# andrpac/alphazero-gnn

Hardware: AMD Instinct MI355X
Metric: board-state evals/sec (GNN fwd) + self-play games/sec, Connect4, 1/2/4/8 GPU (higher is better)
Workload: dtype f32 (fp16x2 row-scaled split, 3 products: output_transform GEMMs and the trunk's conv2 split each fp32 operand row, power-of-two scaled, into 2 fp16 terms, 3 fp16 MFMA products, fp32 accumulate; ~22-bit operands: tests/test_gpu_trained.py holds pi / v / log pi to 1e-5 of float64 and of the reference; 1 GPU; Connect4 (reference 7x7+pass board) Connect4GNN predict_with_gnn per-board fwd: trunk -> output_transform -> heads, batch of random boards per GPU; global_batch=512, batch_per_gpu=512, feature_dim=3136, parallelism=dp1 (independent shards, no collective)

## Files before the change

### alphazero-gnn_amd/csrc/az_gemm.hip

```cpp
#include <stdio.h>
#include <stdlib.h>
#include <string.h>

#include <algorithm>
#include <atomic>
#include <mutex>
#include <type_traits>
#include <utility>
#include <unordered_map>
#include <vector>

#include "az_common.h"
#include "az_x3.h"
#include "az_heads.h"
#include "az_trunk_split.h"

namespace az {

struct GemmArgs {
  int M, N, K;
  const float* A; int lda;
  const float* A2; int lda2; int K0;
  const int* a_rows;
  const float* B; int ldb;
// ... 3450 lines not shown
      } else {
        f = mt % q.am + q.am * ((col >> 7) % q.an);
        b = q.bf;
        W = q.am * q.an * q.KT;
      }
      const int np = csk_block_of((f + 1) * q.KT - 1, b, W) - csk_block_of(f * q.KT, b, W) + 1;
      for (int pc = 0; pc < np; ++pc)
#pragma unroll
        for (int a = 0; a < HS; ++a) s[a] += st[(cb * he.mp + pc) * HS + a];
    }
  } else {
    if (row >= M) return;
    for (int t = lane; t < P; t += 64)
#pragma unroll
      for (int a = 0; a < HS; ++a) s[a] += src[(size_t)t * HS + a];
  }
#pragma unroll
  for (int a = 0; a < HS; ++a) {
    float v = s[a];
    v += dpp_mov<0xB1>(v);
    v += dpp_mov<0x4E>(v);
    v += dpp_mov<0x141>(v);
    v += dpp_mov<0x140>(v);
    s[a] = (__builtin_bit_cast(float, __builtin_amdgcn_readlane(__builtin_bit_cast(int, v), 0)) +
            __builtin_bit_cast(float, __builtin_amdgcn_readlane(__builtin_bit_cast(int, v), 16)) +
            __builtin_bit_cast(float, __builtin_amdgcn_readlane(__builtin_bit_cast(int, v), 32)) +
            __builtin_bit_cast(float, __builtin_amdgcn_readlane(__builtin_bit_cast(int, v), 48)));
  }
  if (lane != 0) return;
  const int A = he.A;
  float l[8];
  float mx = -INFINITY;
#pragma unroll
  for (int a = 0; a < 8; ++a)
    if (a < A) {
      l[a] = s[a] + he.bp[a];
      mx = fmaxf(mx, l[a]);
    }
  float se = 0.f;
#pragma unroll
  for (int a = 0; a < 8; ++a)
    if (a < A) se += expf(l[a] - mx);
  const float lse = logf(se);
#pragma unroll
  for (int a = 0; a < 8; ++a)
    if (a < A) {
      const float o = (l[a] - mx) - lse;
      he.logp[(size_t)row * A + a] = o;
      if (he.pi) he.pi[(size_t)row * A + a] = expf(o);
    }
  he.v[row] = tanhf(s[8] + he.bv[0]);
}

__global__ __launch_bounds__(256) void c4_w2_frag_kernel(const float* __restrict__ w2,
                                                         float* __restrict__ frag) {
  const int i = blockIdx.x * 256 + threadIdx.x;
  if (i >= 18432) return;
  const int e = i & 3, lane = (i >> 2) & 63, q = (i >> 8) % 18, nt = i / (18 * 256);
  const int st = 4 * q + e, tap = st >> 3, j = st & 7;
  const int co = 16 * nt + (lane & 15), ci = 8 * (lane >> 4) + j;
  frag[i] = w2[co * 288 + ci * 9 + tap];
}

const float* conv2_frags(const float* w2, hipStream_t s) {
  if (!weights_registered(w2, 64, 288, 288)) return nullptr;
  const long gen = g_wgen.load();
  std::lock_guard<std::mutex> lk(g_wmu);
  WScaleEntry* e = wcache_entry(w2, 64, 288, 288);
  if (!e) return nullptr;
  if (!e->frags[0]) {
    if (hipMalloc(&e->frags[0], (size_t)2 * 18432 * sizeof(float)) != hipSuccess) {
      e->frags[0] = nullptr;
      return nullptr;
    }
    e->frags[1] = e->frags[0] + 18432;
    e->fgen = 0;
  }
  if (e->fgen == gen) return e->frags[e->fcur];
  const int nxt = e->fcur ^ 1;
  hipLaunchKernelGGL(c4_w2_frag_kernel, dim3(72), dim3(256), 0, s, w2, e->frags[nxt]);
  if (hipStreamSynchronize(s) != hipSuccess) return nullptr;
  e->fcur = nxt;
  e->fgen = gen;
  return e->frags[nxt];
}

constexpr int COMPOSE_JB = 4;
__global__ __launch_bounds__(1024) void compose_heads_kernel(
    const float* __restrict__ w2, const float* __restrict__ b2, const float* __restrict__ wp,
    const float* __restrict__ bp, const float* __restrict__ wv, const float* __restrict__ bv,
    int F, int A, double* __restrict__ part, float* __restrict__ out) {
  __shared__ double sh[3][16][64];
  const int lane = threadIdx.x & 63;
  const int g = __builtin_amdgcn_readfirstlane((int)(threadIdx.x >> 6));
  if ((int)blockIdx.x == (F + 63) / 64) {
    if (blockIdx.y != 0) return;
    double* ps = &sh[0][0][0];
    double* ps2 = ps + 9 * 256;
    const int t = threadIdx.x;
    if (t < 256) {
      double acc[9];
#pragma unroll
      for (int a = 0; a < 9; ++a) acc[a] = 0.0;
      for (int j = t; j < F; j += 256) {
        const double b = (double)b2[j];
#pragma unroll
        for (int a = 0; a < 8; ++a)
          if (a < A) acc[a] += (double)wp[(size_t)a * F + j] * b;
        acc[8] += (double)wv[j] * b;
      }
#pragma unroll
      for (int a = 0; a < 9; ++a) ps[a * 256 + t] = acc[a];
    }
    __syncthreads();
    if (t < 9 * 16) {
      const int a = t >> 4, q = t & 15;
      double s = 0.0;
      for (int i = 0; i < 16; ++i) s += ps[a * 256 + q * 16 + i];
      ps2[a * 16 + q] = s;
    }
    __syncthreads();
    if (t < 9 && (t < A || t == 8)) {
      double s = 0.0;
      for (int q = 0; q < 16; ++q) s += ps2[t * 16 + q];
      const int row = t == 8 ? A : t;
      out[(size_t)(A + 1) * F + row] = (float)(s + (double)(t == 8 ? bv[0] : bp[t]));
    }
    return;
  }
  const int k = blockIdx.x * 64 + lane;
  const bool kin = k < F;
  const int kc = kin ? k : F - 1;
  double acc[9];
// ... 767 lines not shown
```

### alphazero-gnn_amd/csrc/az_trunk.hip

```cpp
#include <stdlib.h>

#include <algorithm>
#include "az_common.h"
#include "az_heads.h"
#include "az_trunk_split.h"
#include "az_x3.h"

namespace az {

#ifdef AZ_TRUNK_SELFCHECK
__device__ unsigned* g_trunk_chk;
#endif

template <int NB, bool REGW>
constexpr int trunk_union_floats() {
  constexpr int after = NB <= 4 ? NB * 3136 : NB * C1_FLOATS_PER_BOARD;
  return REGW || after >= W2S_FLOATS ? after : W2S_FLOATS;
}

template <int NB, bool REGW>
constexpr int trunk_waves_per_eu() { return REGW && NB <= 3 ? 4 : 1; }
template <int NB, bool REGW>
constexpr int trunk_blocks_per_cu() { return REGW && NB <= 3 ? 2 : 1; }

struct TrunkHeads {
  const float* wp; const float* bp; int A; const float* wv; const float* bv;
  float* logp; float* pi; float* v;
};

template <int NB>
__device__ __forceinline__ void trunk_rows_heads(const float* ob, int nb, int b0,
                                                 const TrunkHeads& hd) {
  constexpr int AMAX = 8, PW = AMAX + 1, K = 3136, NCH = (K + HEADS_KC - 1) / HEADS_KC;
  __shared__ float part[NB][NCH][PW];
  __shared__ float hsm[NB][PW];
  const int tid = threadIdx.x, lane = tid & 63, wave = tid >> 6;
  const int A = hd.A;
  const f32x4 z = {0.f, 0.f, 0.f, 0.f};
  static_assert(NCH <= 16, "two chunks per wave");
  auto load_w = [&](int c, f32x4 (&w)[AMAX + 1], bool& kin, int& kc) {
    const int k = c * HEADS_KC + lane * 4;
    kin = k < K;
    kc = kin ? k : 0;
#pragma unroll
    for (int a = 0; a < AMAX; ++a)
      w[a] = *reinterpret_cast<const f32x4*>(hd.wp + (size_t)min(a, A - 1) * K + kc);
    w[AMAX] = *reinterpret_cast<const f32x4*>(hd.wv + kc);
  };
  auto chunk = [&](int c, f32x4 (&w)[AMAX + 1], bool kin, int kc) {
#pragma unroll
    for (int a = 0; a < AMAX; ++a) w[a] = (a < A && kin) ? w[a] : z;
    w[AMAX] = kin ? w[AMAX] : z;
    float ps[NB], vs[NB];
#pragma unroll
    for (int b = 0; b < NB; ++b) {
      const f32x4 x = kin && b < nb ? *reinterpret_cast<const f32x4*>(ob + b * K + kc) : z;
      float pv[AMAX];
#pragma unroll
      for (int a = 0; a < AMAX; ++a)
        pv[a] = fmaf(x[3], w[a][3], fmaf(x[2], w[a][2], fmaf(x[1], w[a][1], x[0] * w[a][0])));
      ps[b] = wave_multi_sum<AMAX>(pv);
      vs[b] = wave_sum_x(
          fmaf(x[3], w[AMAX][3], fmaf(x[2], w[AMAX][2], fmaf(x[1], w[AMAX][1], x[0] * w[AMAX][0]))));
    }
    const int a = lane >> 3;
#pragma unroll
    for (int b = 0; b < NB; ++b) {
      if (b < nb && (lane & 7) == 0 && a < A) part[b][c][a] = ps[b];
      if (b < nb && lane == 0) part[b][c][A] = vs[b];
    }
  };
  f32x4 w0[AMAX + 1], w1[AMAX + 1];
  bool kin0, kin1 = false;
  int kc0, kc1 = 0;
  const bool two = wave + 8 < NCH;
  load_w(wave, w0, kin0, kc0);
  if (two) load_w(wave + 8, w1, kin1, kc1);
  chunk(wave, w0, kin0, kc0);
  if (two) chunk(wave + 8, w1, kin1, kc1);
  __syncthreads();
  if (tid < NB * PW) {
    const int b = tid / PW, a = tid % PW;
    if (b < nb && a <= A) {
      float s = 0.f;
      for (int c = 0; c < NCH; ++c) s += part[b][c][a];
      hsm[b][a] = s;
    }
  }
  __syncthreads();
  if (tid < nb) {
    const int row = b0 + tid;
    float l[AMAX];
    float mx = -INFINITY;
#pragma unroll
    for (int a = 0; a < AMAX; ++a)
      if (a < A) {
        l[a] = hsm[tid][a] + hd.bp[a];
        mx = fmaxf(mx, l[a]);
      }
    float se = 0.f;
#pragma unroll
    for (int a = 0; a < AMAX; ++a)
      if (a < A) se += expf(l[a] - mx);
    const float lse = logf(se);
#pragma unroll
    for (int a = 0; a < AMAX; ++a)
      if (a < A) {
        const float o = (l[a] - mx) - lse;
        hd.logp[(size_t)row * A + a] = o;
        if (hd.pi) hd.pi[(size_t)row * A + a] = expf(o);
      }
    hd.v[row] = tanhf(hsm[tid][A] + hd.bv[0]);
  }
}

template <int NB, bool HEADS = false, bool REGW = false>
__device__ __forceinline__ void c4_trunk_tile(const int8_t* __restrict__ boards, int B,
                                              const float* __restrict__ w1,
                                              const float* __restrict__ b1,
                                              const float* __restrict__ w2,
                                              const float* __restrict__ b2,
                                              float* __restrict__ feat, float* un,
                                              unsigned short* __restrict__ apl = nullptr,
                                              float* __restrict__ asc = nullptr,
                                              const float* __restrict__ w2f = nullptr,
                                              const TrunkHeads* hd = nullptr) {
  static_assert(!HEADS || NB <= 4, "HEADS: the rows staged in LDS");
  float* const ob = un;
  constexpr int P = 49, PP = 81, CI = 32;
  constexpr int NT = TTILES[NB];
  constexpr bool STAGE = NB <= 4;
  __shared__ float bd[NB * PP + 1];
  __shared__ __attribute__((aligned(16))) float c1s[STAGE ? NB * C1_FLOATS_PER_BOARD : 4];
  float* const c1 = STAGE ? c1s : un;
  __shared__ float w1s[CI * 9 + CI + 1];
  __shared__ float c1wmax[NB][8];
  __shared__ float c1inv[NB];
  const int tid = threadIdx.x;
  const int b0 = blockIdx.x * NB;
  const int nb = min(NB, B - b0);
  const int lane = tid & 63, wave = tid >> 6;
  const int nt = wave & 3, mh = wave >> 2;
  const int h = lane >> 4, c16 = lane & 15;
  const int co = nt * 16 + c16;
  const uint16_t* const rows = trunk_rows<NB>();
  constexpr int NW2 = 64 * 72 / 512;
  f32x4v wst[NW2];
  float breg[72];
  if constexpr (REGW) {
#pragma unroll
    for (int q = 0; q < 18; ++q) {
      const f32x4v v = reinterpret_cast<const f32x4v*>(w2f)[(nt * 18 + q) * 64 + lane];
#pragma unroll
      for (int e = 0; e < 4; ++e) breg[4 * q + e] = v[e];
    }
  } else {
#pragma unroll
    for (int j = 0; j < NW2; ++j) wst[j] = reinterpret_cast<const f32x4v*>(w2)[tid + 512 * j];
  }
  constexpr int NBD = (NB * PP + 511) / 512;
  int8_t bdv[NBD];
  bool bdin[NBD];
#pragma unroll
  for (int j = 0; j < NBD; ++j) {
    const int i = tid + 512 * j;
    const int b = i / PP, pp = i % PP, px = pp / 9, py = pp % 9;
    bdin[j] = i < NB * PP && b < nb && px >= 1 && px <= 7 && py >= 1 && py <= 7;
    bdv[j] = boards[bdin[j] ? (size_t)(b0 + b) * P + (px - 1) * 7 + (py - 1) : (size_t)b0 * P];
  }
  const float w1v = tid < CI * 9 ? w1[tid] : b1[min(tid - CI * 9, CI - 1)];
  const float bias = b2[co];
  __builtin_amdgcn_sched_barrier(0);
  if constexpr (!REGW) {
#pragma unroll
    for (int j = 0; j < NW2; ++j) {
      const int i = tid + 512 * j;
      float* d = un + (i / 72) * W2S_STRIDE + (i % 72) * 4;
      d[0] = wst[j][0]; d[1] = wst[j][1]; d[2] = wst[j][2]; d[3] = wst[j][3];
    }
  }
#pragma unroll
  for (int j = 0; j < NBD; ++j)
    bd[min(tid + 512 * j, NB * PP)] = bdin[j] ? (float)bdv[j] : 0.f;
  w1s[min(tid, CI * 9 + CI)] = w1v;
  __syncthreads();
  if constexpr (!REGW) {
#pragma unroll
    for (int s = 0; s < 72; ++s) {
      const int tap = s >> 3, ci = 8 * h + (s & 7);
      breg[s] = un[co * W2S_STRIDE + ci * 9 + (tap / 3) * 3 + (tap % 3)];
    }
  }
  bf16x8 bh[9], bl[9];
  const float iw = w2_planes(breg, bh, bl);
  if constexpr (!STAGE && !REGW) __syncthreads();
  constexpr int NI = NB * PP * 4, NIT = (NI + 511) / 512;
  float cv[NIT][8];
  float cm[NB];
#pragma unroll
  for (int b = 0; b < NB; ++b) cm[b] = 0.f;
#pragma unroll
  for (int it = 0; it < NIT; ++it) {
    const int i = tid + 512 * it;
    if (i < NI) {
      const int b = i / (PP * 4), r = i - b * (PP * 4);
      conv1_octet(w1s, bd + b * PP, r >> 2, r & 3, cv[it]);
      const float m = octet_max(cv[it]);
#pragma unroll
      for (int q = 0; q < NB; ++q)
        if (q == b) cm[q] = fmaxf(cm[q], m);
    }
  }
#pragma unroll
  for (int b = 0; b < NB; ++b) {
#pragma unroll
    for (int o = 32; o > 0; o >>= 1) cm[b] = fmaxf(cm[b], __shfl_xor(cm[b], o));
    if (lane == 0) c1wmax[b][wave] = cm[b];
  }
  __syncthreads();
#pragma unroll
  for (int it = 0; it < NIT; ++it) {
    const int i = tid + 512 * it;
    if (i < NI) {
      const int b = i / (PP * 4), r = i - b * (PP * 4);
      float mx = c1wmax[b][0];
#pragma unroll
      for (int w = 1; w < 8; ++w) mx = fmaxf(mx, c1wmax[b][w]);
      float inv;
      const float sa = h3_scale(mx, H3_TA, &inv);
      c1_store(c1 + b * C1_FLOATS_PER_BOARD, r >> 2, r & 3, cv[it], sa);
      if (r == 0) c1inv[b] = inv;
    }
  }
  __syncthreads();
#ifdef AZ_TRUNK_SELFCHECK
  auto c1_check = [&](int phase, int i) {
    if (i >= NI || !g_trunk_chk) return;
    const int b = i / (PP * 4), r = i - b * (PP * 4);
    float v[8], v2[8];
    conv1_octet(w1s, bd + b * PP, r >> 2, r & 3, v);
    asm volatile("" ::: "memory");
    conv1_octet(w1s, bd + b * PP, r >> 2, r & 3, v2);
    float mx = c1wmax[b][0];
    for (int w = 1; w < 8; ++w) mx = fmaxf(mx, c1wmax[b][w]);
    float inv;
    const float sa = h3_scale(mx, H3_TA, &inv);
    u32x4 o[2];
    split2s(f32x4{v[0], v[1], v[2], v[3]}, f32x4{v[4], v[5], v[6], v[7]}, sa, o);
    const u32x4* u = reinterpret_cast<const u32x4*>(c1 + b * C1_FLOATS_PER_BOARD) +
                     C1_UNITS_PER_POS * (r >> 2) + (r & 3);
    const u32x4 x0 = u[0], x1 = u[4];
    int nbad = 0, nconv = 0;
    for (int e = 0; e < 4; ++e) nbad += (x0[e] != o[0][e]) + (x1[e] != o[1][e]);
    for (int e = 0; e < 8; ++e) nconv += __float_as_uint(v[e]) != __float_as_uint(v2[e]);
    if (nbad || nconv) {
      const unsigned k = atomicAdd(g_trunk_chk, 1u);
      if (k < 2048) {
        unsigned* d = g_trunk_chk + 64 + 48 * k;
        d[0] = blockIdx.x; d[1] = tid; d[2] = i; d[3] = phase;
        d[4] = nbad; d[5] = nconv;
        d[6] = __builtin_amdgcn_s_getreg((4) | (0 << 6) | ((32 - 1) << 11));
        d[7] = __float_as_uint(sa);
        for (int e = 0; e < 4; ++e) {
          d[8 + e] = x0[e]; d[12 + e] = x1[e];
          d[16 + e] = o[0][e]; d[20 + e] = o[1][e];
        }
        for (int e = 0; e < 8; ++e) {
          d[24 + e] = __float_as_uint(v[e]);
          d[32 + e] = __float_as_uint(v2[e]);
        }
      }
    }
  };
#pragma unroll
  for (int it = 0; it < NIT; ++it) c1_check(0, tid + 512 * it);
  c1_check(1, (tid + 192) % (NIT * 512));
#endif

  const u32x4* const c1u = reinterpret_cast<const u32x4*>(c1);
  auto a_unit = [&](int mt) { return mt < NT ? c1_row_unit(rows[16 * mt + c16] & 0x7fff, h) : h; };
  float bm[NB];
#pragma unroll
  for (int b = 0; b < NB; ++b) bm[b] = 0.f;
  auto store_tile = [&](int mt, const f32x4v& acc) {
#pragma unroll
    for (int r = 0; r < 4; ++r) {
      const int e = rows[16 * mt + h * 4 + r];
      const int b = (e & 0x7fff) / P, p = (e & 0x7fff) - P * ((e & 0x7fff) / P);
      if (!(e & 0x8000) && b < nb) {
        const float v = acc[r] * (c1inv[b] * iw) + bias;
        const float o = v > 0.f ? v : 0.f;
        if constexpr (STAGE) {
          ob[b * 3136 + co * P + p] = o;
#pragma unroll
          for (int q = 0; q < NB; ++q)
            if (q == b) bm[q] = fmaxf(bm[q], o);
        } else {
          feat[(size_t)(b0 + b) * 3136 + co * P + p] = o;
        }
      }
    }
  };
  for (int mt = mh; mt < NT; mt += 4) {
    const int u0 = a_unit(mt), u1 = a_unit(mt + 2);
    f32x4v acc0 = {0.f, 0.f, 0.f, 0.f}, acc1 = {0.f, 0.f, 0.f, 0.f};
#pragma unroll
    for (int tap = 0; tap < 9; ++tap) {
      const int off = c1_tap_units(tap);
      const u32x4 ah0 = c1u[u0 + off], al0 = c1u[u0 + off + 4];
      const u32x4 ah1 = c1u[u1 + off], al1 = c1u[u1 + off + 4];
      acc0 = conv2_step(ah0, al0, bh[tap], bl[tap], acc0);
      acc1 = conv2_step(ah1, al1, bh[tap], bl[tap], acc1);
    }
    store_tile(mt, acc0);
    if (mt + 2 < NT) store_tile(mt + 2, acc1);
  }
  if constexpr (STAGE) {
    __shared__ float wmax[NB][8];
    if (apl) {
#pragma unroll
      for (int b = 0; b < NB; ++b) {
#pragma unroll
        for (int o = 32; o > 0; o >>= 1) bm[b] = fmaxf(bm[b], __shfl_xor(bm[b], o));
        if (lane == 0) wmax[b][wave] = bm[b];
      }
    }
    __syncthreads();
#ifdef AZ_TRUNK_SELFCHECK
#pragma unroll
    for (int it = 0; it < NIT; ++it) c1_check(2, tid + 512 * it);
#endif
    f32x4v* dst = feat ? reinterpret_cast<f32x4v*>(feat + (size_t)b0 * 3136) : nullptr;
    const f32x4v* src = reinterpret_cast<const f32x4v*>(ob);
    if (!apl) {
      for (int i = tid; i < nb * 784; i += 512) dst[i] = src[i];
      return;
    }
    for (int ch = tid; ch < nb * 392; ch += 512) {
      const int b = ch / 392, c = ch - b * 392;
      float mx = wmax[b][0];
#pragma unroll
      for (int w = 1; w < 8; ++w) mx = fmaxf(mx, wmax[b][w]);
      float inv;
      const float sc = h3_scale(mx, H3_TA, &inv);
      const f32x4v lo = src[2 * ch], hi = src[2 * ch + 1];
      if (dst) {
        dst[2 * ch] = lo;
        dst[2 * ch + 1] = hi;
      }
      u32x4 o[2];
      split2s(__builtin_bit_cast(f32x4, lo), __builtin_bit_cast(f32x4, hi), sc, o);
      *reinterpret_cast<u32x4*>(apl + p2_chunk(b0 + b, c, 0, 3136)) = o[0];
      *reinterpret_cast<u32x4*>(apl + p2_chunk(b0 + b, c, 1, 3136)) = o[1];
      if (c == 0) {
        asc[b0 + b] = sc;
        asc[B + b0 + b] = inv;
      }
    }
    if constexpr (HEADS) trunk_rows_heads<NB>(ob, nb, b0, *hd);
  }
}

#define AZ_TRUNK_LB(NB_, REGW_)                                                                  \
  __attribute__((amdgpu_flat_work_group_size(1, 512),                                            \
                 amdgpu_waves_per_eu(trunk_waves_per_eu<NB_, REGW_>())))
template <int NB, bool REGW = false>
__global__ AZ_TRUNK_LB(NB, REGW) void c4_trunk_kernel(const int8_t* __restrict__ boards, int B,
                                                      const float* __restrict__ w1,
                                                      const float* __restrict__ b1,
                                                      const float* __restrict__ w2,
                                                      const float* __restrict__ b2,
                                                      float* __restrict__ feat,
                                                      const float* __restrict__ w2f = nullptr) {
  __shared__ __attribute__((aligned(16))) float un[trunk_union_floats<NB, REGW>()];
  c4_trunk_tile<NB, false, REGW>(boards, B, w1, b1, w2, b2, feat, un, nullptr, nullptr, w2f);
}

template <int NB, bool HEADS = false, bool REGW = false>
__global__ AZ_TRUNK_LB(NB, REGW) void c4_trunk_split_a_kernel(
    const int8_t* __restrict__ boards, int B, const float* __restrict__ w1,
    const float* __restrict__ b1, const float* __restrict__ w2, const float* __restrict__ b2,
    float* __restrict__ feat, unsigned short* __restrict__ apl, float* __restrict__ asc,
    const float* __restrict__ w2f = nullptr, TrunkHeads hd = {}) {
  static_assert(NB <= 4, "the A split reads the LDS staging tile");
  __shared__ __attribute__((aligned(16))) float un[trunk_union_floats<NB, REGW>()];
  c4_trunk_tile<NB, HEADS, REGW>(boards, B, w1, b1, w2, b2, feat, un, apl, asc, w2f, &hd);
}

template <bool IN_I8>
__global__ __launch_bounds__(256) void conv3x3_relu_kernel(const void* __restrict__ in_, int B,
                                                          int Cin, int H, int W,
                                                          const float* __restrict__ w,
                                                          const float* __restrict__ b, int Cout,
                                                          int pad, float* __restrict__ out) {
  const int Ho = H + 2 * pad - 2, Wo = W + 2 * pad - 2;
  const long total = (long)B * Cout * Ho * Wo;
  for (long idx = blockIdx.x * 256L + threadIdx.x; idx < total; idx += (long)gridDim.x * 256) {
    const int xo = idx % Wo, yo = (idx / Wo) % Ho, co = (idx / ((long)Wo * Ho)) % Cout;
    const long bi = idx / ((long)Wo * Ho * Cout);
    float s = 0.f;
    for (int ci = 0; ci < Cin; ++ci) {
#pragma unroll
      for (int kh = 0; kh < 3; ++kh) {
        const int yi = yo + kh - pad;
        if (yi < 0 || yi >= H) continue;
#pragma unroll
        for (int kw = 0; kw < 3; ++kw) {
          const int xi = xo + kw - pad;
          if (xi < 0 || xi >= W) continue;
          const long ii = ((bi * Cin + ci) * H + yi) * W + xi;
          const float iv = IN_I8 ? (float)static_cast<const int8_t*>(in_)[ii]
                                 : static_cast<const float*>(in_)[ii];
          s = fmaf(w[((co * Cin + ci) * 3 + kh) * 3 + kw], iv, s);
        }
      }
    }
    s += b[co];
    out[idx] = s > 0.f ? s : 0.f;
  }
}

constexpr int HEADS_ROWS = 16;

template <int AMAX>
__global__ __launch_bounds__(256) void heads_partial_kernel(
    const float* __restrict__ hp, int ldhp, const float* __restrict__ hv, int ldhv, int B, int K,
    const float* __restrict__ wp, int A, const float* __restrict__ wv, float* __restrict__ part) {
  const int c = blockIdx.x;
  const int r0 = blockIdx.y * HEADS_ROWS;
  const int lane = threadIdx.x & 63, wave = threadIdx.x >> 6;
  const int k = c * HEADS_KC + lane * 4;
  const bool kin = k < K;
  const int kc = kin ? k : 0;
  constexpr int RPW = HEADS_ROWS / 4;
  f32x4 xs[RPW], ys[RPW];
  if (hv == hp && ldhv == ldhp) {
#pragma unroll
    for (int i = 0; i < RPW; ++i) {
      const int row = min(r0 + wave + 4 * i, B - 1);
// ... 355 lines not shown
      if (h && kin && r0 + i < B) *reinterpret_cast<f32x4*>(h + (size_t)(r0 + i) * K + k) = x;
      xs[i] = x;
      ys[i] = x;
    }
  });
}

template <int AMAX, int R>
__global__ __launch_bounds__(1024) void heads_rowsw_kernel(
    const float* __restrict__ hp, int ldhp, const float* __restrict__ hv, int ldhv, int B, int K,
    const float* __restrict__ wp, int A, const float* __restrict__ wv,
    const float* __restrict__ bp, const float* __restrict__ bv, float* __restrict__ logp,
    float* __restrict__ pi, float* __restrict__ v) {
  heads_rowsw_body<AMAX, R>(B, K, wp, A, wv, bp, bv, logp, pi, v,
                            [&](int r0, int kc, bool, int, f32x4 (&xs)[R], f32x4 (&ys)[R]) {
#pragma unroll
    for (int i = 0; i < R; ++i) {
      const int row = min(r0 + i, B - 1);
      xs[i] = *reinterpret_cast<const f32x4*>(hp + (size_t)row * ldhp + kc);
      ys[i] = *reinterpret_cast<const f32x4*>(hv + (size_t)row * ldhv + kc);
    }
  });
}

__global__ __launch_bounds__(256) void c4_trunk_split_kernel(
    const int8_t* __restrict__ boards, const float* __restrict__ w1, const float* __restrict__ b1,
    const float* __restrict__ w2, const float* __restrict__ b2, float* __restrict__ feat) {
  __shared__ TrunkSplitSmem sm;
  c4_trunk_split_block(boards, w1, b1, w2, b2, feat, blockIdx.x, blockIdx.y, sm);
}

template <int NB>
__global__ __launch_bounds__(512) void c4_trunk_heads_kernel(
    const int8_t* __restrict__ boards, int B, const float* __restrict__ w1,
    const float* __restrict__ b1, const float* __restrict__ w2, const float* __restrict__ b2,
    float* __restrict__ feat, const float* __restrict__ wp, const float* __restrict__ bp, int A,
    const float* __restrict__ wv, const float* __restrict__ bv, float* __restrict__ logp,
    float* __restrict__ pi, float* __restrict__ v) {
  __shared__ __attribute__((aligned(16))) float ob[trunk_union_floats<NB, false>()];
  __shared__ float part[HEADS_ROWS_MAXC * 9];
  __shared__ float sm[9];
  c4_trunk_tile<NB>(boards, B, w1, b1, w2, b2, feat, ob);
  const int b0 = blockIdx.x * NB, nb = min(NB, B - b0);
  for (int b = 0; b < nb; ++b)
    heads_row_block<8, 8>(ob + b * 3136, ob + b * 3136, 3136, wp, A, wv, bp, bv, b0 + b, logp, pi, v,
                       part, sm);
}

}

using namespace az;

namespace az {
const float* conv2_frags(const float* w2, hipStream_t s);

static int c4_trunk_launch(const int8_t* boards, int B, const float* conv1_w,
                           const float* conv1_b, const float* conv2_w, const float* conv2_b,
                           float* feat, unsigned short* apl, float* asc, bool* split,
                           hipStream_t s, const TrunkHeads* heads = nullptr,
                           bool* heads_done = nullptr, bool feat_optional = false) {
  static const char* env = tuning_env("AZ_TRUNK_NB");
  static int cus = 0;
  if (cus <= 0) {
    int dev = 0, n = 0;
    cus = (hipGetDevice(&dev) == hipSuccess &&
           hipDeviceGetAttribute(&n, hipDeviceAttributeMultiprocessorCount, dev) == hipSuccess &&
           n > 0) ? n : 256;
  }
  static const bool no_frag = tuning_env("AZ_TRUNK_NO_W2F") != nullptr;
  const float* w2f = B > 8 && !no_frag ? conv2_frags(conv2_w, s) : nullptr;
  const bool regw = w2f != nullptr;
  int nbk = 0;
  if (B > 8) {
    static const float ra[9] = {0.f, 4.3f, 5.f, 7.3f, 2.5f, 1.5f, 0.f, 0.f, 0.5f};
    static const float rb[9] = {0.f, 4.1f, 5.95f, 7.3f, 14.3f, 22.f, 26.f, 29.7f, 32.5f};
    static const float ua[9] = {0.f, 2.f, 2.6f, 3.7f, 3.5f, 3.f, 0.f, 0.f, 0.f};
    static const float ub[9] = {0.f, 7.6f, 10.8f, 11.8f, 15.5f, 22.f, 26.f, 30.5f, 33.f};
    const float* ta = regw ? ra : ua;
    const float* tb = regw ? rb : ub;
    float best = 0.f;
    for (int nb = 1; nb <= 8; ++nb) {
      const long k = ((long)(B + nb - 1) / nb + cus - 1) / cus;
      const float t = ta[nb] + (float)k * tb[nb] + (apl && nb > 4 ? 0.0038f * B : 0.f);
      if (nb == 1 || t < best) best = t, nbk = nb;
    }
  }
  if (regw && apl && asc && !heads && B > cus && B <= 2 * cus) nbk = 1;
  if (env) nbk = atoi(env);
  const bool sa = apl && asc && nbk >= 1 && nbk <= 4;
  if (split) *split = sa;
  const bool hk = sa && heads && heads->A >= 1 && heads->A <= 8;
  if (heads_done) *heads_done = hk;
  float* const feat_sa = feat_optional && sa && (!heads || hk) ? nullptr : feat;
#ifdef AZ_TUNING
  static const char* env_dyn = tuning_env("AZ_TRUNK_DYN_LDS");
  const size_t dyn = env_dyn ? (size_t)atol(env_dyn) : 0;
#else
  constexpr size_t dyn = 0;
#endif
#define AZ_TRUNK_RW(NB_, RW_)                                                                    \
  if (hk) hipLaunchKernelGGL((c4_trunk_split_a_kernel<NB_, true, RW_>),                          \
                             dim3((B + NB_ - 1) / NB_), dim3(512), dyn, s, boards, B, conv1_w,  \
                             conv1_b, conv2_w, conv2_b, feat_sa, apl, asc, w2f, *heads);         \
  else if (sa) hipLaunchKernelGGL((c4_trunk_split_a_kernel<NB_, false, RW_>),                    \
                                  dim3((B + NB_ - 1) / NB_), dim3(512), dyn, s, boards, B,      \
                                  conv1_w, conv1_b, conv2_w, conv2_b, feat_sa, apl, asc, w2f,   \
                                  TrunkHeads{});                                                 \
  else hipLaunchKernelGGL((c4_trunk_kernel<NB_, RW_>), dim3((B + NB_ - 1) / NB_), dim3(512),    \
                          dyn, s, boards, B, conv1_w, conv1_b, conv2_w, conv2_b, feat, w2f);
#define AZ_TRUNK(NB_)                                                                            \
  if (regw) { AZ_TRUNK_RW(NB_, true) } else { AZ_TRUNK_RW(NB_, false) }
#define AZ_TRUNK_BIG(NB_)                                                                        \
  if (regw) hipLaunchKernelGGL((c4_trunk_kernel<NB_, true>), dim3((B + NB_ - 1) / NB_),         \
                               dim3(512), dyn, s, boards, B, conv1_w, conv1_b, conv2_w, conv2_b, \
                               feat, w2f);                                                       \
  else hipLaunchKernelGGL((c4_trunk_kernel<NB_, false>), dim3((B + NB_ - 1) / NB_), dim3(512),  \
                          dyn, s, boards, B, conv1_w, conv1_b, conv2_w, conv2_b, feat, nullptr);
  switch (nbk) {
    case 8: AZ_TRUNK_BIG(8) break;
    case 7: AZ_TRUNK_BIG(7) break;
    case 6: AZ_TRUNK_BIG(6) break;
    case 5: AZ_TRUNK_BIG(5) break;
    case 4: AZ_TRUNK(4) break;
    case 3: AZ_TRUNK(3) break;
    case 2: AZ_TRUNK(2) break;
    case 0:
      hipLaunchKernelGGL(c4_trunk_split_kernel, dim3(B, 4), dim3(256), 0, s, boards, conv1_w,
                         conv1_b, conv2_w, conv2_b, feat);
      break;
    default: AZ_TRUNK(1)
  }
#undef AZ_TRUNK
#undef AZ_TRUNK_RW
#undef AZ_TRUNK_BIG
  return check_launch("c4_trunk_kernel");
}
}

#ifdef AZ_TRUNK_SELFCHECK
extern "C" int az_debug_trunk_chk(void* log) {
  return hipMemcpyToSymbol(HIP_SYMBOL(g_trunk_chk), &log, sizeof(log)) == hipSuccess ? 0 : -1;
}
#endif

extern "C" int az_c4_trunk_fwd(const int8_t* boards, int B, const float* conv1_w,
                               const float* conv1_b, const float* conv2_w, const float* conv2_b,
                               float* feat, void* stream) {
  AZ_REQUIRE(B >= 0, AZ_EINVAL, "az_c4_trunk_fwd: B=%d", B);
  if (B == 0) return AZ_OK;
  AZ_REQUIRE(boards && conv1_w && conv1_b && conv2_w && conv2_b && feat, AZ_EINVAL,
             "az_c4_trunk_fwd: null pointer");
  return c4_trunk_launch(boards, B, conv1_w, conv1_b, conv2_w, conv2_b, feat, nullptr, nullptr,
                         nullptr, as_stream(stream));
}

extern "C" int az_conv3x3_relu_fwd(const void* in, int in_int8, int B, int Cin, int H, int W,
                                   const float* w, const float* b, int Cout, int pad, float* out,
                                   void* stream) {
  AZ_REQUIRE(B >= 0 && Cin > 0 && Cout > 0 && H >= 3 - 2 * pad && W >= 3 - 2 * pad &&
                 (pad == 0 || pad == 1),
             AZ_EINVAL, "az_conv3x3_relu_fwd: bad shape");
  if (B == 0) return AZ_OK;
  AZ_REQUIRE(in && w && b && out, AZ_EINVAL, "az_conv3x3_relu_fwd: null pointer");
  AZ_REQUIRE(!in_int8 || Cin == 1, AZ_EINVAL, "az_conv3x3_relu_fwd: int8 input needs Cin=1");
  const long total = (long)B * Cout * (H + 2 * pad - 2) * (W + 2 * pad - 2);
  const int blocks = (int)std::min<long>((total + 255) / 256, 8192);
  hipStream_t s = as_stream(stream);
  if (in_int8)
    hipLaunchKernelGGL(conv3x3_relu_kernel<true>, dim3(blocks), dim3(256), 0, s, in, B, Cin, H, W,
                       w, b, Cout, pad, out);
  else
    hipLaunchKernelGGL(conv3x3_relu_kernel<false>, dim3(blocks), dim3(256), 0, s, in, B, Cin, H,
                       W, w, b, Cout, pad, out);
  return check_launch("conv3x3_relu_kernel");
}

namespace az {
int gemv1_with_side_heads(const az_gemm_desc* d, const SideHeads* h, hipStream_t s);
int c4_leaf_fwd(const az_c4_eval* e, const int8_t* boards, int B, float* pi, float* v, float* gpi,
                float* gv, hipStream_t s);
int gemm_f32(const az_gemm_desc* d, hipStream_t s);
int gemm_f32_partial(const az_gemm_desc* d, hipStream_t s, int* splits_out, const PreSplitA* pre,
                     const HeadsEpi* he = nullptr, bool* heads_done = nullptr);
int splitk_reduce(const az_gemm_desc* d, int splits, hipStream_t s);
bool gemm_p2_certain(const az_gemm_desc* d, hipStream_t s);
int splitk_reduce_split(const az_gemm_desc* d, int splits, unsigned short* planes, float* sc,
                        hipStream_t s, bool write_c = true);
bool gemm_p2_weights(const float* w, int n, int k, int ld);
const float* conv2_frags(const float* w2, hipStream_t s);
size_t composed_heads_scratch_bytes(int F, int A);
const float* composed_heads(const float* w2, const float* b2, const float* wp, const float* bp,
                            const float* wv, const float* bv, int F, int A, float* scratch,
                            hipStream_t s);

static size_t align256(size_t b) { return (b + 255) & ~size_t(255); }

constexpr int COMPOSED_HEADS_MIN_B = 65;
static bool composed_heads_shape(int B, int A, bool want_y) {
  static const bool off = tuning_env("AZ_NO_COMPOSED_HEADS") != nullptr;
  return !off && !want_y && A >= 1 && A <= 8 && B >= COMPOSED_HEADS_MIN_B;
}
static size_t composed_heads_bytes(int F, int A) {
  return align256(composed_heads_scratch_bytes(F, A));
}

struct PreRegion {
  unsigned short* planes;
  float* sc;
  size_t bytes;
};
static size_t pre_region_bytes(int B, int F) {
  return align256((size_t)4 * B * F) + align256((size_t)8 * B) + 256;
}
static PreRegion pre_region(void* ws, size_t ws_bytes, int B, int F, size_t reserved) {
  const size_t need = pre_region_bytes(B, F);
  if (!ws || ws_bytes < reserved + need) return {nullptr, nullptr, 0};
  char* base = static_cast<char*>(ws) + (ws_bytes - need + 255) / 256 * 256;
  return {reinterpret_cast<unsigned short*>(base),
          reinterpret_cast<float*>(base + align256((size_t)4 * B * F)), need};
}
}

extern "C" size_t az_heads_ws_bytes(int B, int K, int A) {
  return (size_t)((K + HEADS_KC - 1) / HEADS_KC) * (size_t)B * (size_t)(A + 1) * 4;
}

template <int AMAX>
static void launch_heads(const float* hp, int ldhp, const float* hv, int ldhv, int B, int K,
                         const float* wp, const float* bp, int A, const float* wv,
                         const float* bv, float* logp, float* pi, float* v, float* part,
                         hipStream_t s) {
  const int nchunks = (K + HEADS_KC - 1) / HEADS_KC;
  static const bool two_pass = tuning_env("AZ_HEADS_TWOPASS") != nullptr;
  if (B <= HEADS_ROWS_MAXB && nchunks <= HEADS_ROWS_MAXC && !two_pass) {
    hipLaunchKernelGGL(heads_rows_kernel<AMAX>, dim3(B), dim3(512), 0, s, hp, ldhp, hv, ldhv, K,
                       wp, A, wv, bp, bv, logp, pi, v);
    return;
  }
  static const char* env_r = tuning_env("AZ_HEADS_R");
  int R = B > 768 ? 4 : 2;
  if (env_r) R = atoi(env_r);
  if (AMAX == 8 && nchunks <= 16 && !two_pass && B <= 8192 && (R == 2 || R == 4 || R == 8)) {
// ... 409 lines not shown
```

Before: 9.280 million board evals/s.

## Precompute conv2 bf16 weight planes once and add 4-wave single-board trunk variant

The cached conv2 weight buffer now holds the weights already split into bf16 high/low planes plus a per-lane inverse scale. The trunk kernel loads these planes directly, after conv1, instead of loading fp32 fragments and re-splitting them in every block. A new 4-wave (256-thread) variant for one board per block is chosen by a cost model when it beats the 8-wave configurations, and the tile cost tables for the non-heads path are retuned. Optional timestamp instrumentation is added behind a compile flag. The 4-wave path halves per-block parallelism in conv1 and conv2 and relies on the tuned cost constants to pick it well.

```diff
diff --git a/alphazero-gnn_amd/csrc/az_gemm.hip b/alphazero-gnn_amd/csrc/az_gemm.hip
--- a/alphazero-gnn_amd/csrc/az_gemm.hip
+++ b/alphazero-gnn_amd/csrc/az_gemm.hip
@@ -3526,33 +3526,43 @@
   he.v[row] = tanhf(s[8] + he.bv[0]);
 }
 
-__global__ __launch_bounds__(256) void c4_w2_frag_kernel(const float* __restrict__ w2,
-                                                         float* __restrict__ frag) {
-  const int i = blockIdx.x * 256 + threadIdx.x;
-  if (i >= 18432) return;
-  const int e = i & 3, lane = (i >> 2) & 63, q = (i >> 8) % 18, nt = i / (18 * 256);
-  const int st = 4 * q + e, tap = st >> 3, j = st & 7;
-  const int co = 16 * nt + (lane & 15), ci = 8 * (lane >> 4) + j;
-  frag[i] = w2[co * 288 + ci * 9 + tap];
-}
-
-const float* conv2_frags(const float* w2, hipStream_t s) {
+constexpr int W2P_UNITS = 4 * 18 * 64;
+constexpr int W2P_FLOATS = W2P_UNITS * 4 + 4 * 64;
+__global__ __launch_bounds__(64) void c4_w2_planes_kernel(const float* __restrict__ w2,
+                                                          float* __restrict__ out) {
+  const int nt = blockIdx.x, lane = threadIdx.x;
+  const int co = 16 * nt + (lane & 15), h = lane >> 4;
+  float breg[72];
+#pragma unroll
+  for (int st = 0; st < 72; ++st) breg[st] = w2[co * 288 + (8 * h + (st & 7)) * 9 + (st >> 3)];
+  bf16x8 bh[9], bl[9];
+  const float iw = w2_planes(breg, bh, bl);
+  u32x4* const u = reinterpret_cast<u32x4*>(out);
+#pragma unroll
+  for (int t = 0; t < 9; ++t) {
+    u[(nt * 18 + t) * 64 + lane] = __builtin_bit_cast(u32x4, bh[t]);
+    u[(nt * 18 + 9 + t) * 64 + lane] = __builtin_bit_cast(u32x4, bl[t]);
+  }
+  out[W2P_UNITS * 4 + nt * 64 + lane] = iw;
+}
+
+const float* conv2_planes(const float* w2, hipStream_t s) {
   if (!weights_registered(w2, 64, 288, 288)) return nullptr;
   const long gen = g_wgen.load();
   std::lock_guard<std::mutex> lk(g_wmu);
   WScaleEntry* e = wcache_entry(w2, 64, 288, 288);
   if (!e) return nullptr;
   if (!e->frags[0]) {
-    if (hipMalloc(&e->frags[0], (size_t)2 * 18432 * sizeof(float)) != hipSuccess) {
+    if (hipMalloc(&e->frags[0], (size_t)2 * W2P_FLOATS * sizeof(float)) != hipSuccess) {
       e->frags[0] = nullptr;
       return nullptr;
     }
-    e->frags[1] = e->frags[0] + 18432;
+    e->frags[1] = e->frags[0] + W2P_FLOATS;
     e->fgen = 0;
   }
   if (e->fgen == gen) return e->frags[e->fcur];
   const int nxt = e->fcur ^ 1;
-  hipLaunchKernelGGL(c4_w2_frag_kernel, dim3(72), dim3(256), 0, s, w2, e->frags[nxt]);
+  hipLaunchKernelGGL(c4_w2_planes_kernel, dim3(4), dim3(64), 0, s, w2, e->frags[nxt]);
   if (hipStreamSynchronize(s) != hipSuccess) return nullptr;
   e->fcur = nxt;
   e->fgen = gen;
diff --git a/alphazero-gnn_amd/csrc/az_trunk.hip b/alphazero-gnn_amd/csrc/az_trunk.hip
--- a/alphazero-gnn_amd/csrc/az_trunk.hip
+++ b/alphazero-gnn_amd/csrc/az_trunk.hip
@@ -12,16 +12,29 @@
 __device__ unsigned* g_trunk_chk;
 #endif
 
+#ifdef AZ_TRUNK_STAMPS
+__device__ unsigned long long* g_trunk_stamps;
+#define AZ_TSTAMP(k)                                                                       \
+  do {                                                                                     \
+    const unsigned long long t_ = __builtin_amdgcn_s_memrealtime();                        \
+    if (g_trunk_stamps && (threadIdx.x & 63) == 0)                                         \
+      g_trunk_stamps[((size_t)blockIdx.x * 8 + (threadIdx.x >> 6)) * 8 + (k)] = t_;        \
+  } while (0)
+#else
+#define AZ_TSTAMP(k)
+#endif
+
 template <int NB, bool REGW>
 constexpr int trunk_union_floats() {
   constexpr int after = NB <= 4 ? NB * 3136 : NB * C1_FLOATS_PER_BOARD;
   return REGW || after >= W2S_FLOATS ? after : W2S_FLOATS;
 }
 
+template <bool W4>
+constexpr int trunk_waves() { return W4 ? 4 : 8; }
+
 template <int NB, bool REGW>
 constexpr int trunk_waves_per_eu() { return REGW && NB <= 3 ? 4 : 1; }
-template <int NB, bool REGW>
-constexpr int trunk_blocks_per_cu() { return REGW && NB <= 3 ? 2 : 1; }
 
 struct TrunkHeads {
   const float* wp; const float* bp; int A; const float* wv; const float* bv;
@@ -114,7 +127,7 @@
   }
 }
 
-template <int NB, bool HEADS = false, bool REGW = false>
+template <int NB, bool HEADS = false, bool REGW = false, bool W4 = false>
 __device__ __forceinline__ void c4_trunk_tile(const int8_t* __restrict__ boards, int B,
                                               const float* __restrict__ w1,
                                               const float* __restrict__ b1,
@@ -126,15 +139,18 @@
                                               const float* __restrict__ w2f = nullptr,
                                               const TrunkHeads* hd = nullptr) {
   static_assert(!HEADS || NB <= 4, "HEADS: the rows staged in LDS");
+  static_assert(!W4 || (REGW && NB == 1 && !HEADS),
+                "4 waves: the cached planes, one board per block, no heads (8 waves there)");
   float* const ob = un;
   constexpr int P = 49, PP = 81, CI = 32;
   constexpr int NT = TTILES[NB];
   constexpr bool STAGE = NB <= 4;
+  constexpr int NW = trunk_waves<W4>(), T = 64 * NW;
   __shared__ float bd[NB * PP + 1];
   __shared__ __attribute__((aligned(16))) float c1s[STAGE ? NB * C1_FLOATS_PER_BOARD : 4];
   float* const c1 = STAGE ? c1s : un;
   __shared__ float w1s[CI * 9 + CI + 1];
-  __shared__ float c1wmax[NB][8];
+  __shared__ float c1wmax[NB][NW];
   __shared__ float c1inv[NB];
   const int tid = threadIdx.x;
   const int b0 = blockIdx.x * NB;
@@ -144,64 +160,69 @@
   const int h = lane >> 4, c16 = lane & 15;
   const int co = nt * 16 + c16;
   const uint16_t* const rows = trunk_rows<NB>();
-  constexpr int NW2 = 64 * 72 / 512;
-  f32x4v wst[NW2];
-  float breg[72];
-  if constexpr (REGW) {
-#pragma unroll
-    for (int q = 0; q < 18; ++q) {
-      const f32x4v v = reinterpret_cast<const f32x4v*>(w2f)[(nt * 18 + q) * 64 + lane];
-#pragma unroll
-      for (int e = 0; e < 4; ++e) breg[4 * q + e] = v[e];
-    }
-  } else {
-#pragma unroll
-    for (int j = 0; j < NW2; ++j) wst[j] = reinterpret_cast<const f32x4v*>(w2)[tid + 512 * j];
-  }
-  constexpr int NBD = (NB * PP + 511) / 512;
+  AZ_TSTAMP(0);
+  constexpr int NBD = (NB * PP + T - 1) / T;
   int8_t bdv[NBD];
   bool bdin[NBD];
 #pragma unroll
   for (int j = 0; j < NBD; ++j) {
-    const int i = tid + 512 * j;
+    const int i = tid + T * j;
     const int b = i / PP, pp = i % PP, px = pp / 9, py = pp % 9;
     bdin[j] = i < NB * PP && b < nb && px >= 1 && px <= 7 && py >= 1 && py <= 7;
     bdv[j] = boards[bdin[j] ? (size_t)(b0 + b) * P + (px - 1) * 7 + (py - 1) : (size_t)b0 * P];
   }
-  const float w1v = tid < CI * 9 ? w1[tid] : b1[min(tid - CI * 9, CI - 1)];
+  constexpr int NW1 = (CI * 9 + CI + T - 1) / T;
+  float w1v[NW1];
+#pragma unroll
+  for (int j = 0; j < NW1; ++j) {
+    const int i = tid + T * j;
+    w1v[j] = i < CI * 9 ? w1[i] : b1[min(i - CI * 9, CI - 1)];
+  }
   const float bias = b2[co];
+  constexpr int NW2 = REGW ? 1 : 64 * 72 / T;
+  f32x4v wst[NW2];
+  bf16x8 bh[9], bl[9];
+  float iw;
+  if constexpr (!REGW) {
+#pragma unroll
+    for (int j = 0; j < NW2; ++j) wst[j] = reinterpret_cast<const f32x4v*>(w2)[tid + T * j];
+  }
   __builtin_amdgcn_sched_barrier(0);
   if constexpr (!REGW) {
 #pragma unroll
     for (int j = 0; j < NW2; ++j) {
-      const int i = tid + 512 * j;
+      const int i = tid + T * j;
       float* d = un + (i / 72) * W2S_STRIDE + (i % 72) * 4;
       d[0] = wst[j][0]; d[1] = wst[j][1]; d[2] = wst[j][2]; d[3] = wst[j][3];
     }
   }
 #pragma unroll
   for (int j = 0; j < NBD; ++j)
-    bd[min(tid + 512 * j, NB * PP)] = bdin[j] ? (float)bdv[j] : 0.f;
-  w1s[min(tid, CI * 9 + CI)] = w1v;
+    bd[min(tid + T * j, NB * PP)] = bdin[j] ? (float)bdv[j] : 0.f;
+#pragma unroll
+  for (int j = 0; j < NW1; ++j)
+    w1s[min(tid + T * j, CI * 9 + CI)] = w1v[j];
   __syncthreads();
+  AZ_TSTAMP(1);
   if constexpr (!REGW) {
+    float breg[72];
 #pragma unroll
     for (int s = 0; s < 72; ++s) {
       const int tap = s >> 3, ci = 8 * h + (s & 7);
       breg[s] = un[co * W2S_STRIDE + ci * 9 + (tap / 3) * 3 + (tap % 3)];
     }
-  }
-  bf16x8 bh[9], bl[9];
-  const float iw = w2_planes(breg, bh, bl);
+    iw = w2_planes(breg, bh, bl);
+  }
+  AZ_TSTAMP(2);
   if constexpr (!STAGE && !REGW) __syncthreads();
-  constexpr int NI = NB * PP * 4, NIT = (NI + 511) / 512;
+  constexpr int NI = NB * PP * 4, NIT = (NI + T - 1) / T;
   float cv[NIT][8];
   float cm[NB];
 #pragma unroll
   for (int b = 0; b < NB; ++b) cm[b] = 0.f;
 #pragma unroll
   for (int it = 0; it < NIT; ++it) {
-    const int i = tid + 512 * it;
+    const int i = tid + T * it;
     if (i < NI) {
       const int b = i / (PP * 4), r = i - b * (PP * 4);
       conv1_octet(w1s, bd + b * PP, r >> 2, r & 3, cv[it]);
@@ -211,6 +232,18 @@
         if (q == b) cm[q] = fmaxf(cm[q], m);
     }
   }
+  AZ_TSTAMP(3);
+  if constexpr (REGW) {
+    __builtin_amdgcn_sched_barrier(0);
+    const u32x4* const pu = reinterpret_cast<const u32x4*>(w2f) + nt * 18 * 64 + lane;
+#pragma unroll
+    for (int t = 0; t < 9; ++t) {
+      bh[t] = __builtin_bit_cast(bf16x8, pu[t * 64]);
+      bl[t] = __builtin_bit_cast(bf16x8, pu[(9 + t) * 64]);
+    }
+    iw = w2f[4 * 18 * 64 * 4 + nt * 64 + lane];
+    __builtin_amdgcn_sched_barrier(0);
+  }
 #pragma unroll
   for (int b = 0; b < NB; ++b) {
 #pragma unroll
@@ -220,12 +253,12 @@
   __syncthreads();
 #pragma unroll
   for (int it = 0; it < NIT; ++it) {
-    const int i = tid + 512 * it;
+    const int i = tid + T * it;
     if (i < NI) {
       const int b = i / (PP * 4), r = i - b * (PP * 4);
       float mx = c1wmax[b][0];
 #pragma unroll
-      for (int w = 1; w < 8; ++w) mx = fmaxf(mx, c1wmax[b][w]);
+      for (int w = 1; w < NW; ++w) mx = fmaxf(mx, c1wmax[b][w]);
       float inv;
       const float sa = h3_scale(mx, H3_TA, &inv);
       c1_store(c1 + b * C1_FLOATS_PER_BOARD, r >> 2, r & 3, cv[it], sa);
@@ -233,6 +266,7 @@
     }
   }
   __syncthreads();
+  AZ_TSTAMP(4);
 #ifdef AZ_TRUNK_SELFCHECK
   auto c1_check = [&](int phase, int i) {
     if (i >= NI || !g_trunk_chk) return;
@@ -242,7 +276,7 @@
     asm volatile("" ::: "memory");
     conv1_octet(w1s, bd + b * PP, r >> 2, r & 3, v2);
     float mx = c1wmax[b][0];
-    for (int w = 1; w < 8; ++w) mx = fmaxf(mx, c1wmax[b][w]);
+    for (int w = 1; w < NW; ++w) mx = fmaxf(mx, c1wmax[b][w]);
     float inv;
     const float sa = h3_scale(mx, H3_TA, &inv);
     u32x4 o[2];
@@ -273,8 +307,8 @@
     }
   };
 #pragma unroll
-  for (int it = 0; it < NIT; ++it) c1_check(0, tid + 512 * it);
-  c1_check(1, (tid + 192) % (NIT * 512));
+  for (int it = 0; it < NIT; ++it) c1_check(0, tid + T * it);
+  c1_check(1, (tid + 192) % (NIT * T));
 #endif
 
   const u32x4* const c1u = reinterpret_cast<const u32x4*>(c1);
@@ -282,10 +316,10 @@
   float bm[NB];
 #pragma unroll
   for (int b = 0; b < NB; ++b) bm[b] = 0.f;
-  auto store_tile = [&](int mt, const f32x4v& acc) {
+  auto store_tile = [&](const uint16_t (&er)[4], const f32x4v& acc) {
 #pragma unroll
     for (int r = 0; r < 4; ++r) {
-      const int e = rows[16 * mt + h * 4 + r];
+      const int e = er[r];
       const int b = (e & 0x7fff) / P, p = (e & 0x7fff) - P * ((e & 0x7fff) / P);
       if (!(e & 0x8000) && b < nb) {
         const float v = acc[r] * (c1inv[b] * iw) + bias;
@@ -301,8 +335,15 @@
       }
     }
   };
-  for (int mt = mh; mt < NT; mt += 4) {
+  for (int mt0 = 0; mt0 < NT; mt0 += 4)
+  for (int mt = mt0 + mh; mt < min(mt0 + 2, NT); mt += NW / 4) {
     const int u0 = a_unit(mt), u1 = a_unit(mt + 2);
+    uint16_t er0[4], er1[4];
+#pragma unroll
+    for (int r = 0; r < 4; ++r) {
+      er0[r] = rows[16 * mt + h * 4 + r];
+      er1[r] = rows[16 * (mt + 2 < NT ? mt + 2 : mt) + h * 4 + r];
+    }
     f32x4v acc0 = {0.f, 0.f, 0.f, 0.f}, acc1 = {0.f, 0.f, 0.f, 0.f};
 #pragma unroll
     for (int tap = 0; tap < 9; ++tap) {
@@ -312,11 +353,12 @@
       acc0 = conv2_step(ah0, al0, bh[tap], bl[tap], acc0);
       acc1 = conv2_step(ah1, al1, bh[tap], bl[tap], acc1);
     }
-    store_tile(mt, acc0);
-    if (mt + 2 < NT) store_tile(mt + 2, acc1);
-  }
+    store_tile(er0, acc0);
+    if (mt + 2 < NT) store_tile(er1, acc1);
+  }
+  AZ_TSTAMP(5);
   if constexpr (STAGE) {
-    __shared__ float wmax[NB][8];
+    __shared__ float wmax[NB][NW];
     if (apl) {
 #pragma unroll
       for (int b = 0; b < NB; ++b) {
@@ -326,21 +368,22 @@
       }
     }
     __syncthreads();
+    AZ_TSTAMP(6);
 #ifdef AZ_TRUNK_SELFCHECK
 #pragma unroll
-    for (int it = 0; it < NIT; ++it) c1_check(2, tid + 512 * it);
+    for (int it = 0; it < NIT; ++it) c1_check(2, tid + T * it);
 #endif
     f32x4v* dst = feat ? reinterpret_cast<f32x4v*>(feat + (size_t)b0 * 3136) : nullptr;
     const f32x4v* src = reinterpret_cast<const f32x4v*>(ob);
     if (!apl) {
-      for (int i = tid; i < nb * 784; i += 512) dst[i] = src[i];
+      for (int i = tid; i < nb * 784; i += T) dst[i] = src[i];
       return;
     }
-    for (int ch = tid; ch < nb * 392; ch += 512) {
+    for (int ch = tid; ch < nb * 392; ch += T) {
       const int b = ch / 392, c = ch - b * 392;
       float mx = wmax[b][0];
 #pragma unroll
-      for (int w = 1; w < 8; ++w) mx = fmaxf(mx, wmax[b][w]);
+      for (int w = 1; w < NW; ++w) mx = fmaxf(mx, wmax[b][w]);
       float inv;
       const float sc = h3_scale(mx, H3_TA, &inv);
       const f32x4v lo = src[2 * ch], hi = src[2 * ch + 1];
@@ -357,6 +400,7 @@
         asc[B + b0 + b] = inv;
       }
     }
+    AZ_TSTAMP(7);
     if constexpr (HEADS) trunk_rows_heads<NB>(ob, nb, b0, *hd);
   }
 }
@@ -364,7 +408,7 @@
 #define AZ_TRUNK_LB(NB_, REGW_)                                                                  \
   __attribute__((amdgpu_flat_work_group_size(1, 512),                                            \
                  amdgpu_waves_per_eu(trunk_waves_per_eu<NB_, REGW_>())))
-template <int NB, bool REGW = false>
+template <int NB, bool REGW = false, bool W4 = false>
 __global__ AZ_TRUNK_LB(NB, REGW) void c4_trunk_kernel(const int8_t* __restrict__ boards, int B,
                                                       const float* __restrict__ w1,
                                                       const float* __restrict__ b1,
@@ -373,10 +417,10 @@
                                                       float* __restrict__ feat,
                                                       const float* __restrict__ w2f = nullptr) {
   __shared__ __attribute__((aligned(16))) float un[trunk_union_floats<NB, REGW>()];
-  c4_trunk_tile<NB, false, REGW>(boards, B, w1, b1, w2, b2, feat, un, nullptr, nullptr, w2f);
-}
-
-template <int NB, bool HEADS = false, bool REGW = false>
+  c4_trunk_tile<NB, false, REGW, W4>(boards, B, w1, b1, w2, b2, feat, un, nullptr, nullptr, w2f);
+}
+
+template <int NB, bool HEADS = false, bool REGW = false, bool W4 = false>
 __global__ AZ_TRUNK_LB(NB, REGW) void c4_trunk_split_a_kernel(
     const int8_t* __restrict__ boards, int B, const float* __restrict__ w1,
     const float* __restrict__ b1, const float* __restrict__ w2, const float* __restrict__ b2,
@@ -384,7 +428,7 @@
     const float* __restrict__ w2f = nullptr, TrunkHeads hd = {}) {
   static_assert(NB <= 4, "the A split reads the LDS staging tile");
   __shared__ __attribute__((aligned(16))) float un[trunk_union_floats<NB, REGW>()];
-  c4_trunk_tile<NB, HEADS, REGW>(boards, B, w1, b1, w2, b2, feat, un, apl, asc, w2f, &hd);
+  c4_trunk_tile<NB, HEADS, REGW, W4>(boards, B, w1, b1, w2, b2, feat, un, apl, asc, w2f, &hd);
 }
 
 template <bool IN_I8>
@@ -846,7 +890,7 @@
 using namespace az;
 
 namespace az {
-const float* conv2_frags(const float* w2, hipStream_t s);
+const float* conv2_planes(const float* w2, hipStream_t s);
 
 static int c4_trunk_launch(const int8_t* boards, int B, const float* conv1_w,
                            const float* conv1_b, const float* conv2_w, const float* conv2_b,
@@ -862,25 +906,30 @@
            n > 0) ? n : 256;
   }
   static const bool no_frag = tuning_env("AZ_TRUNK_NO_W2F") != nullptr;
-  const float* w2f = B > 8 && !no_frag ? conv2_frags(conv2_w, s) : nullptr;
+  const float* w2f = B > 8 && !no_frag ? conv2_planes(conv2_w, s) : nullptr;
   const bool regw = w2f != nullptr;
   int nbk = 0;
+  bool w4 = false;
   if (B > 8) {
-    static const float ra[9] = {0.f, 4.3f, 5.f, 7.3f, 2.5f, 1.5f, 0.f, 0.f, 0.5f};
-    static const float rb[9] = {0.f, 4.1f, 5.95f, 7.3f, 14.3f, 22.f, 26.f, 29.7f, 32.5f};
+    static const float ra[9] = {0.f, 3.4f, 5.4f, 6.f, 4.f, 1.5f, 0.f, 0.f, 0.5f};
+    static const float rb[9] = {0.f, 2.86f, 4.64f, 6.f, 12.6f, 22.f, 26.f, 29.7f, 32.5f};
     static const float ua[9] = {0.f, 2.f, 2.6f, 3.7f, 3.5f, 3.f, 0.f, 0.f, 0.f};
     static const float ub[9] = {0.f, 7.6f, 10.8f, 11.8f, 15.5f, 22.f, 26.f, 30.5f, 33.f};
-    const float* ta = regw ? ra : ua;
-    const float* tb = regw ? rb : ub;
+    static const float ha[9] = {0.f, 4.3f, 5.f, 7.3f, 2.5f, 1.5f, 0.f, 0.f, 0.5f};
+    static const float hb[9] = {0.f, 4.1f, 5.95f, 7.3f, 14.3f, 22.f, 26.f, 29.7f, 32.5f};
+    const float* ta = regw ? (heads ? ha : ra) : ua;
+    const float* tb = regw ? (heads ? hb : rb) : ub;
     float best = 0.f;
     for (int nb = 1; nb <= 8; ++nb) {
       const long k = ((long)(B + nb - 1) / nb + cus - 1) / cus;
       const float t = ta[nb] + (float)k * tb[nb] + (apl && nb > 4 ? 0.0038f * B : 0.f);
       if (nb == 1 || t < best) best = t, nbk = nb;
     }
-  }
-  if (regw && apl && asc && !heads && B > cus && B <= 2 * cus) nbk = 1;
-  if (env) nbk = atoi(env);
+    static const bool no_w4 = tuning_env("AZ_TRUNK_NO_W4") != nullptr;
+    if (regw && !heads && !no_w4 && 5.1f + 2.24f * (float)((B + cus - 1) / cus) < best)
+      nbk = 1, w4 = true;
+  }
+  if (env) nbk = atoi(env), w4 = w4 && nbk == 1;
   const bool sa = apl && asc && nbk >= 1 && nbk <= 4;
   if (split) *split = sa;
   const bool hk = sa && heads && heads->A >= 1 && heads->A <= 8;
@@ -892,18 +941,20 @@
 #else
   constexpr size_t dyn = 0;
 #endif
-#define AZ_TRUNK_RW(NB_, RW_)                                                                    \
-  if (hk) hipLaunchKernelGGL((c4_trunk_split_a_kernel<NB_, true, RW_>),                          \
+#define AZ_TRUNK_RW(NB_, RW_, W4_)                                                               \
+  constexpr int TT = 64 * trunk_waves<W4_>();                                                    \
+  if (hk) hipLaunchKernelGGL((c4_trunk_split_a_kernel<NB_, true, RW_, false>),                   \
                              dim3((B + NB_ - 1) / NB_), dim3(512), dyn, s, boards, B, conv1_w,  \
                              conv1_b, conv2_w, conv2_b, feat_sa, apl, asc, w2f, *heads);         \
-  else if (sa) hipLaunchKernelGGL((c4_trunk_split_a_kernel<NB_, false, RW_>),                    \
-                                  dim3((B + NB_ - 1) / NB_), dim3(512), dyn, s, boards, B,      \
+  else if (sa) hipLaunchKernelGGL((c4_trunk_split_a_kernel<NB_, false, RW_, W4_>),               \
+                                  dim3((B + NB_ - 1) / NB_), dim3(TT), dyn, s, boards, B,       \
                                   conv1_w, conv1_b, conv2_w, conv2_b, feat_sa, apl, asc, w2f,   \
                                   TrunkHeads{});                                                 \
-  else hipLaunchKernelGGL((c4_trunk_kernel<NB_, RW_>), dim3((B + NB_ - 1) / NB_), dim3(512),    \
-                          dyn, s, boards, B, conv1_w, conv1_b, conv2_w, conv2_b, feat, w2f);
+  else hipLaunchKernelGGL((c4_trunk_kernel<NB_, RW_, W4_>), dim3((B + NB_ - 1) / NB_),          \
+                          dim3(TT), dyn, s, boards, B, conv1_w, conv1_b, conv2_w, conv2_b, feat, \
+                          w2f);
 #define AZ_TRUNK(NB_)                                                                            \
-  if (regw) { AZ_TRUNK_RW(NB_, true) } else { AZ_TRUNK_RW(NB_, false) }
+  if (regw) { AZ_TRUNK_RW(NB_, true, false) } else { AZ_TRUNK_RW(NB_, false, false) }
 #define AZ_TRUNK_BIG(NB_)                                                                        \
   if (regw) hipLaunchKernelGGL((c4_trunk_kernel<NB_, true>), dim3((B + NB_ - 1) / NB_),         \
                                dim3(512), dyn, s, boards, B, conv1_w, conv1_b, conv2_w, conv2_b, \
@@ -922,7 +973,8 @@
       hipLaunchKernelGGL(c4_trunk_split_kernel, dim3(B, 4), dim3(256), 0, s, boards, conv1_w,
                          conv1_b, conv2_w, conv2_b, feat);
       break;
-    default: AZ_TRUNK(1)
+    default:
+      if (regw && w4) { AZ_TRUNK_RW(1, true, true) } else { AZ_TRUNK(1) }
   }
 #undef AZ_TRUNK
 #undef AZ_TRUNK_RW
@@ -930,6 +982,12 @@
   return check_launch("c4_trunk_kernel");
 }
 }
+
+#ifdef AZ_TRUNK_STAMPS
+extern "C" int az_debug_trunk_stamps(void* buf) {
+  return hipMemcpyToSymbol(HIP_SYMBOL(g_trunk_stamps), &buf, sizeof(buf)) == hipSuccess ? 0 : -1;
+}
+#endif
 
 #ifdef AZ_TRUNK_SELFCHECK
 extern "C" int az_debug_trunk_chk(void* log) {
@@ -981,7 +1039,7 @@
 int splitk_reduce_split(const az_gemm_desc* d, int splits, unsigned short* planes, float* sc,
                         hipStream_t s, bool write_c = true);
 bool gemm_p2_weights(const float* w, int n, int k, int ld);
-const float* conv2_frags(const float* w2, hipStream_t s);
+const float* conv2_planes(const float* w2, hipStream_t s);
 size_t composed_heads_scratch_bytes(int F, int A);
 const float* composed_heads(const float* w2, const float* b2, const float* wp, const float* bp,
                             const float* wv, const float* bv, int F, int A, float* scratch,
```

New measurement: 10.02 million board evals/s (median of 6 runs). 1.08x the previous value.
